# aask1357/hilcodec

Hardware: AMD Instinct MI355X
Metric: audio-seconds/sec (xRT) encode+RVQ+decode, 24 kHz batch=256 (higher is better)
Workload: dtype f32

## Files before the change

### hilcodec_amd/csrc/resblock_cfg.h

```cpp
#pragma once
#include <stdlib.h>

#include <atomic>
#include <type_traits>

#include "gemm_core.h"

using namespace hilc;

namespace {

constexpr int DWS = 12;

#ifndef HILC_RES_SHARE2_0
#define HILC_RES_SHARE2_0 0.61
#endif
#ifndef HILC_RES_SHARE3_0
#define HILC_RES_SHARE3_0 0.44
#define HILC_RES_SHARE3_1 0.31
#endif
template <int C, bool STREAM, bool SCARRY_ = false, int NB_ = 1, bool W8_ = false, int DR_ = 0, bool POST_ = false, bool SPEC0_ = false>
struct Cfg {
  static constexpr bool POST = POST_;
  static constexpr bool SPEC0 = SPEC0_;
  static_assert(!SPEC0_ || (C == 64 && (!STREAM || SCARRY_) && !W8_ && DR_ >= 0), "stage-0 input phase: the C = 64 encoder stage in the carry form (four waves, 128-column tiles)");
  static_assert(!POST_ || ((!STREAM || SCARRY_) && DR_ <= 0 && C <= 192 && !W8_), "closing conv: the carry form of a narrow stage (offline, or a hop's runs of whole streams)");
  static constexpr int NB = NB_;
  static constexpr int DR = DR_ > 0 ? DR_ : 0;
  static constexpr int UR = DR_ < 0 ? -DR_ : 0;
  static_assert(DR_ <= 0 || (((DR_ == 2 || DR_ == 4) && (!STREAM || SCARRY_) && C <= 192) || ((!STREAM || SCARRY_) && DR_ == 5 && C == 256) || (!SCARRY_ && DR_ == 8 && C == 512)),
                "down-sampling phase: carry form, r = 2 / 4 (C <= 192) or the wide encoder stages (C = 256: r = 5, offline and the hop's 32-column carry form; C = 512: r = 8, offline and a hop's whole-stream tiles)");
  static constexpr int DCAR = DR_ <= 0 ? 0 : (DR_ == 5 ? 12 : (DR_ == 8 ? 8 : 4));
  static_assert(DR_ >= 0 || ((DR_ == -8 && C >= 512) || (DR_ == -5 && C == 384) || ((DR_ == -4 || DR_ == -2) && C <= 192 && (!STREAM || SCARRY_))),
                "up-sampling phase: 32-column tiles (r = 8: whole streams, or the offline carry form), the C = 384 stage (r = 5) or the carry form (r = 4 / 2)");
  static constexpr int CH = C;
  static constexpr int CB = C / 32;
  static constexpr bool NARROW = C >= 256;
  static constexpr bool N32 = STREAM && SCARRY_ && NARROW;
  static_assert(!N32 || C == 256 || C == 384, "32-column carry form: the C = 256 / C = 384 stages of a hop");
  static constexpr int NCOL = NARROW ? ((C >= 512 || N32) ? 32 : 64) : 128;
  static constexpr int XS = NCOL + ((!STREAM || SCARRY_) ? 8 * NB_ + 2 * DCAR + (POST_ ? 4 : 0) : 0);
  static constexpr bool CARRYMODE = !STREAM || SCARRY_;
  static constexpr int HALO = CARRYMODE ? 0 : ((NARROW && C >= 512) ? 0 : 8);
  static constexpr int TO = NCOL - HALO;
  static constexpr int NW = (N32 && C == 384) ? 12 : ((C >= 192 || W8_) ? 8 : 4);
  static constexpr int NT = 64 * NW;
  static constexpr int RH = NW / (NCOL / 32);
  static constexpr int CBW = CB / RH;
  static constexpr int RPI = 256 / NCOL;
  static constexpr int RSTEP = RPI * NW;
  static constexpr int RW = C / RSTEP;
#ifndef HILC_RES_RB
#define HILC_RES_RB 4
#endif
  static constexpr int RB = HILC_RES_RB;
#ifdef HILC_RES_KP
  static constexpr int KP = HILC_RES_KP;
  static constexpr int DEPTH = HILC_RES_DEPTH;
#else
  static constexpr int KP = C >= 96 ? 4 : 8;
  static constexpr int DEPTH = C >= 256 ? 4 : (C == 128 ? (STREAM ? 2 : 3) : 2);
#endif
#ifndef HILC_RES_MINW
#define HILC_RES_MINW 2
#endif
  static constexpr int MINW = NW >= 8 ? NW / 4 : HILC_RES_MINW;
  static_assert(NW % (NCOL / 32) == 0 && CB % RH == 0 && RW % RB == 0 && C % RSTEP == 0, "tile split");
  static_assert(NB_ >= 1 && NB_ <= 3 && (NB_ == 1 || CARRYMODE || (NARROW && C >= 512)), "a chain needs carries or whole-stream tiles");
};

struct ResBlk {
  const float* w1t;
  const float* dw1_w;
  const float* dw1_b;
  const float* w2t;
  const float* dw2_w;
  const float* dw2_b;
  const float* hist1;
  const float* hist2;
  float* hist1_out;
  float* hist2_out;
  float pre_scale, out_scale;
};

struct ResUp {
  const float* xin;
  const float* tr_w;
  const float* w_lo;
  const float* w_hi;
  const float* bias;
  const float* hist;
  float* hist_out;
  float in_scale;
};

struct ResDown {
  const float* w_lo;
  const float* w_hi;
  const float* dw_w;
  const float* dw_b;
  const float* hist;
  float* hist_out;
  const float* res;
  float* y;
  float in_scale;
};

struct ResPost {
  const float* w;
  const float* bias;
  float* wav;
  const float* hist;
  float* hist_out;
  float in_scale, out_scale;
  int do_tanh;
};

struct ResSpec0 {
  const float* wav;
  const float* dft;
  const float* nyq;
  const float* pw;
  const float* bias;
  const float* pre_w;
  const float* pre_b;
  const float* hist;
  int hist_len;
  float pre_in_scale, mean, stdv, out_scale;
  int normalize;
};

constexpr int POST_CLASSES = 8;

constexpr int MAXBLK = 3;
constexpr int DDS = 12;

struct ResArgs {
  const float* x;
  ResBlk blk[MAXBLK];
  int nblk;
  ResDown dn;
  ResUp up;
  ResPost post;
  ResSpec0 spec;
  long run_tiles;
  float* y;
  int T, tiles;
  int classes;
  unsigned cum[5];
  long total_tiles;
  int B;
  unsigned div_magic, div_shift;
  int* sched;
  unsigned long long* dbg;
};

#ifdef HILC_DEBUG_STAMPS
unsigned long long* g_dbg = nullptr;
#endif

}
```

### hilcodec_amd/csrc/resblock_kernel.h

```cpp
#pragma once
#include "resblock_gemm.h"
#include "stream_gemm.h"

namespace {

struct Cols {
  long b;
  int t;
  int t_in;
  unsigned boff;
  unsigned hoff;
  int head, tail;
};
static_assert(sizeof(Cols) == 32, "no padding");

template <int C, bool STREAM, bool SCARRY = false, int NB = 1, bool W8 = false, int DRU = 0, bool POST = false, bool SPEC0 = false>
__global__ __launch_bounds__((Cfg<C, STREAM, SCARRY, NB, W8, DRU, POST, SPEC0>::NT), (Cfg<C, STREAM, SCARRY, NB, W8, DRU, POST, SPEC0>::MINW)) void resblock_kernel(ResArgs a) {
  using K = Cfg<C, STREAM, SCARRY, NB, W8, DRU, POST, SPEC0>;
  constexpr int DR = K::DR, UR = K::UR;
  using Pipe = WeightPipe<K>;
  constexpr int CBW = K::CBW, NW = K::NW, NT = K::NT, RW = K::RW, RB = K::RB, XS = K::XS, TO = K::TO, RSTEP = K::RSTEP;
  __shared__ __attribute__((aligned(16))) float Xbuf[4 + C * XS];
  constexpr bool DW_RELOAD = NB > 1 && K::NARROW && (4 + C * XS + NB * C * DWS) * 4 > 156 * 1024;
  __shared__ __attribute__((aligned(16))) float DW[(DW_RELOAD ? 1 : NB) * C * DWS];
  constexpr bool DWIDE = DR == 5 || DR == 8;
  __shared__ __attribute__((aligned(16))) float DWD[(DR > 0 && !DWIDE) ? 2 * C * DDS : 4];
  __shared__ __attribute__((aligned(16))) float HS[(STREAM && !K::NARROW) ? 2 * C * 4 : 4];
  __shared__ __attribute__((aligned(16))) float PR[POST ? POST_CLASSES * K::NCOL : 4];
  static_assert(!POST || (K::RPI * K::NW == POST_CLASSES), "a row class of the closing conv = the rows one half-wave walks");
  __shared__ __attribute__((aligned(16))) float SEG[SPEC0 ? (STREAM ? 256 : 192) : 4];
  __shared__ __attribute__((aligned(16))) float SEGS[SPEC0 ? (STREAM ? 256 : 192) : 4];
  float* const X = Xbuf + 4;
  const int tid = threadIdx.x, lane = tid & 63;
  const int wave = __builtin_amdgcn_readfirstlane(tid >> 6);
  constexpr int NCB = K::NCOL / 32;
  const int colblk = wave % NCB;
  const int wclass = wave / NCB;
  const int rowblk0 = wclass * CBW;
#if defined(HILC_DEBUG_WAVE_STAMPS)
  constexpr int WS_MAXB = 48;
  unsigned long long* ws_base = nullptr;
  int ws_k = 0;
#define STAMP(i) do { } while (0)
#define lds_barrier() do {                                                                                          \
    const unsigned long long t0_ = __builtin_amdgcn_s_memtime();                                                   \
    asm volatile("s_waitcnt lgkmcnt(0)" ::: "memory");                                                             \
    const unsigned long long t1_ = __builtin_amdgcn_s_memtime();                                                   \
    asm volatile("s_waitcnt lgkmcnt(0)\n\ts_barrier" ::: "memory");                                                 \
    const unsigned long long t2_ = __builtin_amdgcn_s_memtime();                                                   \
    if (ws_base != nullptr && lane == 0 && ws_k < WS_MAXB - 1) {                                                   \
      ws_base[ws_k * 3] = t0_; ws_base[ws_k * 3 + 1] = t1_; ws_base[ws_k * 3 + 2] = t2_;                           \
    }                                                                                                              \
    ++ws_k;                                                                                                        \
  } while (0)
#elif defined(HILC_DEBUG_STAMPS)
#define STAMP(i) do { if (a.dbg && tid == 0) a.dbg[stamp_tile * 8 + (i)] = __builtin_amdgcn_s_memtime(); } while (0)
  long stamp_tile = blockIdx.x;
#else
#define STAMP(i) do { } while (0)
#endif
  const int T = a.T;
  const int nblk = NB == 1 ? 1 : a.nblk;
  auto load_taps = [&](const ResBlk& bq, float* dst) {
    if constexpr (DW_RELOAD && !STREAM) {
      constexpr int NE = C * DWS;
      static_assert(NE % NT == 0, "whole rounds");
#pragma unroll
      for (int i = 0; i < NE / NT; ++i) {
        const int e = tid + i * NT;
        const int m = e / DWS, j = e - m * DWS;
        const float* src = j < 5 ? bq.dw1_w + (m * 5 + j) : (j == 5 ? bq.dw1_b + m : (j < 11 ? bq.dw2_w + (m * 5 + (j - 6)) : bq.dw2_b + m));
        dst[e] = *src;
      }
    } else if constexpr (DW_RELOAD) {
      constexpr int NE = C * DWS;
      static_assert(NE % NT == 0, "whole rounds");
#pragma unroll 3
      for (int i = 0; i < NE / NT; ++i) {
        const int e = tid + i * NT;
        const int m = e / DWS, j = e - m * DWS;
        const float* src = j < 5 ? bq.dw1_w + (m * 5 + j) : (j == 5 ? bq.dw1_b + m : (j < 11 ? bq.dw2_w + (m * 5 + (j - 6)) : bq.dw2_b + m));
        dst[e] = *src;
      }
    }
  };
  if constexpr (!DW_RELOAD) {
    constexpr int RND = (C + NT - 1) / NT;
    if constexpr (NB == 1 && STREAM) {
      const ResBlk& bq = a.blk[0];
#pragma unroll
      for (int it = 0; it < RND; ++it) {
        const int m = tid + it * NT;
        const int mc = (C % NT == 0 || m < C) ? m : C - 1;
#pragma unroll
        for (int w4 = 0; w4 < DWS / 4; ++w4) {
          float t4[4];
#pragma unroll
          for (int e = 0; e < 4; ++e) {
            const int j = 4 * w4 + e;
            t4[e] = j < 5 ? bq.dw1_w[mc * 5 + j] : (j == 5 ? bq.dw1_b[mc] : (j < 11 ? bq.dw2_w[mc * 5 + (j - 6)] : bq.dw2_b[mc]));
          }
          if (C % NT == 0 || m < C) *reinterpret_cast<f32x4*>(&DW[m * DWS + 4 * w4]) = f32x4{t4[0], t4[1], t4[2], t4[3]};
          __builtin_amdgcn_sched_barrier(0);
        }
      }
    } else {
    float tv[NB][RND][DWS];
#pragma unroll
    for (int q = 0; q < NB; ++q) {
      if (q < nblk) {
        const ResBlk& bq = a.blk[q];
#pragma unroll
        for (int it = 0; it < RND; ++it) {
          const int m = tid + it * NT;
          const int mc = (C % NT == 0 || m < C) ? m : C - 1;
#pragma unroll
          for (int j = 0; j < 5; ++j) tv[q][it][j] = bq.dw1_w[mc * 5 + j];
          tv[q][it][5] = bq.dw1_b[mc];
#pragma unroll
          for (int j = 0; j < 5; ++j) tv[q][it][6 + j] = bq.dw2_w[mc * 5 + j];
          tv[q][it][11] = bq.dw2_b[mc];
        }
      }
    }
#pragma unroll
    for (int q = 0; q < NB; ++q) {
      if (q < nblk) {
#pragma unroll
        for (int it = 0; it < RND; ++it) {
          const int m = tid + it * NT;
          if (C % NT == 0 || m < C) {
#pragma unroll
            for (int w4 = 0; w4 < DWS / 4; ++w4)
              *reinterpret_cast<f32x4*>(&DW[(q * C + m) * DWS + 4 * w4]) =
                  f32x4{tv[q][it][4 * w4], tv[q][it][4 * w4 + 1], tv[q][it][4 * w4 + 2], tv[q][it][4 * w4 + 3]};
          }
        }
      }
    }
    }
  }
  if constexpr (DR > 0 && !DWIDE) {
    constexpr int RND = (2 * C + NT - 1) / NT;
    float tw[RND][2 * DR + 1];
#pragma unroll
    for (int it = 0; it < RND; ++it) {
      const int m = tid + it * NT;
      const int mc = ((2 * C) % NT == 0 || m < 2 * C) ? m : 2 * C - 1;
#pragma unroll
      for (int j = 0; j < 2 * DR; ++j) tw[it][j] = a.dn.dw_w[mc * 2 * DR + j];
      tw[it][2 * DR] = a.dn.dw_b[mc];
    }
#pragma unroll
    for (int it = 0; it < RND; ++it) {
      const int m = tid + it * NT;
      if ((2 * C) % NT == 0 || m < 2 * C) {
#pragma unroll
        for (int j = 0; j < DDS; ++j) DWD[m * DDS + j] = j < 2 * DR ? tw[it][j] : (j == 8 ? tw[it][2 * DR] : 0.f);
      }
    }
  }
  if (tid < 4) Xbuf[tid] = 0.f;
  const int rsub = wave * K::RPI + (K::RPI > 1 ? lane / (K::NCOL / 4) : 0);
  const int c4 = (lane & (K::NCOL / 4 - 1)) * 4;
  [[maybe_unused]] const unsigned row_b = (unsigned)T * 4u;
  [[maybe_unused]] const bool one_head = STREAM && !K::NARROW && T >= K::NCOL;

  auto columns_of = [&](long tile) -> Cols {
    Cols s;
    s.boff = 0; s.hoff = 0; s.head = false; s.tail = false;
    if constexpr (STREAM) {
      const int flat = (int)tile * TO - K::HALO + c4;
      s.t_in = flat >= 0 && flat < a.B * T;
      const unsigned ub = s.t_in ? __umulhi((unsigned)flat, a.div_magic) >> a.div_shift : 0u;
      s.b = ub;
      s.t = s.t_in ? flat - (int)ub * T : 0;
      s.boff = (ub * (unsigned)(C * T) + (unsigned)s.t) * 4u;
      s.hoff = ub * (unsigned)(C * 4);
      s.head = s.t_in && s.t == 0;
      s.tail = s.t_in && c4 >= K::HALO && s.t == T - 4;
    } else {
      s.b = tile / a.tiles;
      s.t = (int)(tile - s.b * a.tiles) * TO + c4;
      s.t_in = s.t >= 0 && s.t < T;
    }
    return s;
  };
  auto xrow = [&](const Cols& s, int m) -> const f32x4* {
    if constexpr (STREAM)
      return reinterpret_cast<const f32x4*>(reinterpret_cast<const char*>(a.x) + (s.boff + (unsigned)m * row_b));
    else
      return reinterpret_cast<const f32x4*>(a.x + s.b * (long)C * T + (long)m * T + (s.t_in ? s.t : 0));
  };
  auto yrow = [&](const Cols& s, int m) -> f32x4* {
    if constexpr (STREAM)
      return reinterpret_cast<f32x4*>(reinterpret_cast<char*>(a.y) + (s.boff + (unsigned)m * row_b));
    else
      return reinterpret_cast<f32x4*>(a.y + s.b * (long)C * T + (long)m * T + s.t);
  };

  [[maybe_unused]] const float* hb0 = a.x;
  [[maybe_unused]] const float* hb1 = a.x;
  [[maybe_unused]] bool hv0 = false, hv1 = false;
  [[maybe_unused]] int blk_off = 0;
  Cols cs;
  const bool lane0 = c4 == 0, lane_last = c4 == K::NCOL - 4;
  auto prev_base = [&](int which) -> lptr_t {
    if constexpr (!K::CARRYMODE) return (lptr_t)(X + rsub * XS + c4 - 4);
    else return lane0 ? (lptr_t)(X + rsub * XS + K::NCOL + which * 4 + blk_off) : (lptr_t)(X + rsub * XS + c4 - 4);
  };
  auto prevs_of = [&](lptr_t pb, int m0, int which, f32x4 (&prev)[K::RB]) {
    if constexpr (!STREAM) {
// ... 505 lines not shown
      carry_out(xp6, 1, cur);
      if constexpr (STREAM) {
        if (cs.tail && !warm && bp.hist2_out != nullptr) {
#pragma unroll
          for (int i = 0; i < RB; ++i)
            *reinterpret_cast<f32x4*>(bp.hist2_out + cs.hoff + (rsub + RSTEP * (i0 + i)) * 4) = cur[i];
        }
      }
#pragma unroll
      for (int i = 0; i < RB; ++i) {
        const int m = rsub + RSTEP * (i0 + i);
        const float v[8] = {prev[i].x, prev[i].y, prev[i].z, prev[i].w, cur[i].x, cur[i].y, cur[i].z, cur[i].w};
        const float w[5] = {wb[i].x, wb[i].y, wc[i].x, wc[i].y, wc[i].z};
        f32x4 o;
#pragma unroll
        for (int e = 0; e < 4; ++e) {
          float s = 0.f;
#pragma unroll
          for (int j = 0; j < 5; ++j) s = fmaf(w[j], v[e + j], s);
          s = __fmul_rn(__fadd_rn(s, wc[i].w), bp.out_scale);
          o[e] = __fadd_rn(s, xr[i0 + i][e]);
        }
        if constexpr (NB == 1 && DR == 0 && !POST) {
          if (out_ok) *yrow(cs, m) = o;
        } else {
          if (last_blk) {
            if (out_ok) *yrow(cs, m) = o;
          } else if (post_blk) {
            *(lvec_t)(xp6 + i * RSTEP * XS) = prologue4v(o, a.post.in_scale, 1);
          } else {
            xr[i0 + i] = o;
          }
        }
      }
      if (UR == 0 && !SPEC0 && last_blk && have_next) {
#pragma unroll
        for (int i = 0; i < RB; ++i) xr[i0 + i] = *xrow(cn, rsub + RSTEP * (i0 + i));
      }
      xp6 += RB * RSTEP * XS;
      pb6 += RB * RSTEP * XS;
      asm volatile("" : "+v"(xp6), "+v"(pb6));
      __builtin_amdgcn_sched_barrier(0);
    }
    STAMP(7);
    lds_barrier();
    if (last_blk) cs = cn;
    }
    if constexpr (POST) {
      const bool have_next = next_tile < run1;
      const Cols cn = columns_of(have_next ? next_tile : tile);
      constexpr int PSLOT = K::NCOL + 8 * NB;
      float part[4] = {0.f, 0.f, 0.f, 0.f};
      lptr_t xq = (lptr_t)(X + rsub * XS + c4);
      lptr_t pq = lane0 ? (lptr_t)(X + rsub * XS + PSLOT) : (lptr_t)(X + rsub * XS + c4 - 4);
      const float* wq = a.post.w + rsub * 5;
      [[maybe_unused]] bool any_head = false;
      [[maybe_unused]] const float* hq = a.post.w;
      [[maybe_unused]] float* hqo = nullptr;
      [[maybe_unused]] bool qtail = false;
      if constexpr (STREAM) {
        const int first = (int)tile * TO, last = first + K::NCOL - 1;
        const unsigned bl = __umulhi((unsigned)last, a.div_magic) >> a.div_shift;
        any_head = (int)bl * T >= first || first % T == 0;
        if (a.post.hist != nullptr) hq = a.post.hist + cs.hoff + rsub * 4;
        qtail = cs.tail && !warm && a.post.hist_out != nullptr;
        if (a.post.hist_out != nullptr) hqo = a.post.hist_out + cs.hoff + rsub * 4;
      }
#pragma nounroll
      for (int i0 = 0; i0 < RW; i0 += RB) {
        f32x4 cur[RB], prev[RB];
        float w[RB][5];
#pragma unroll
        for (int i = 0; i < RB; ++i) {
          cur[i] = *(lvec_t)(xq + i * RSTEP * XS);
          prev[i] = *(lvec_t)(pq + i * RSTEP * XS);
#pragma unroll
          for (int j = 0; j < 5; ++j) w[i][j] = wq[i * RSTEP * 5 + j];
        }
        wq += RB * RSTEP * 5;
        if constexpr (STREAM) {
          if (any_head) {
            f32x4 hv[RB];
#pragma unroll
            for (int i = 0; i < RB; ++i)
              hv[i] = a.post.hist != nullptr ? *reinterpret_cast<const f32x4*>(hq + i * RSTEP * 4) : f32x4{0.f, 0.f, 0.f, 0.f};
#pragma unroll
            for (int i = 0; i < RB; ++i)
#pragma unroll
              for (int e = 0; e < 4; ++e) prev[i][e] = cs.head ? hv[i][e] : prev[i][e];
          }
          if (qtail) {
#pragma unroll
            for (int i = 0; i < RB; ++i) *reinterpret_cast<f32x4*>(hqo + i * RSTEP * 4) = cur[i];
          }
          hq += a.post.hist != nullptr ? RB * RSTEP * 4 : 0;
          hqo += RB * RSTEP * 4;
        }
        if (lane_last) {
#pragma unroll
          for (int i = 0; i < RB; ++i) *(lvec_t)(xq + i * RSTEP * XS + 4 + 8 * NB) = cur[i];
        }
#pragma unroll
        for (int i = 0; i < RB; ++i) {
          const float v[8] = {prev[i].x, prev[i].y, prev[i].z, prev[i].w, cur[i].x, cur[i].y, cur[i].z, cur[i].w};
#pragma unroll
          for (int e = 0; e < 4; ++e)
#pragma unroll
            for (int j = 0; j < 5; ++j) part[e] = fmaf(w[i][j], v[e + j], part[e]);
        }
        xq += RB * RSTEP * XS;
        pq += RB * RSTEP * XS;
        asm volatile("" : "+v"(xq), "+v"(pq));
        __builtin_amdgcn_sched_barrier(0);
      }
      *reinterpret_cast<f32x4*>(&PR[rsub * K::NCOL + c4]) = f32x4{part[0], part[1], part[2], part[3]};
      lds_barrier();
      if (tid < K::NCOL) {
        float sacc = PR[tid];
#pragma unroll
        for (int q = 1; q < POST_CLASSES; ++q) sacc = __fadd_rn(sacc, PR[q * K::NCOL + tid]);
        if (a.post.bias != nullptr) sacc = __fadd_rn(sacc, a.post.bias[0]);
        sacc = __fmul_rn(sacc, a.post.out_scale);
        if (a.post.do_tanh) sacc = tanhf(sacc);
        if constexpr (STREAM) {
          const long flat = (long)tile * TO + tid;
          if (!warm && flat < (long)a.B * T) a.post.wav[flat] = sacc;
        } else {
          const int t = cs.t - c4 + tid;
          if (!warm && t < T) a.post.wav[cs.b * (long)T + t] = sacc;
        }
      }
      cs = cn;
    }
    if constexpr (DR > 0) {
      const ResDown& dn = a.dn;
      const bool have_next = next_tile < run1;
      const Cols cn = columns_of(have_next ? next_tile : tile);
      const float* wd0 = dn.w_lo + (long)wclass * (C * C / K::RH);
      const float* wd1 = dn.w_hi + (long)wclass * (C * C / K::RH);
      asm volatile("" : "+s"(wd0), "+s"(wd1));
      Pipe wp;
      wp.prefetch(wd0, lane);
      auto d0 = [&]() {
        lptr_t xp = (lptr_t)(X + rsub * XS + c4);
#pragma unroll
        for (int i0 = 0; i0 < RW; i0 += RB) {
#pragma unroll
          for (int i = 0; i < RB; ++i)
            *(lvec_t)(xp + i * RSTEP * XS) = prologue4v(zero_unless(cs.t_in, xr[i0 + i]), dn.in_scale, 1);
          xp += RB * RSTEP * XS;
          asm volatile("" : "+v"(xp));
        }
      };
      d0();
      if (!DWIDE && !SPEC0 && have_next) {
#pragma unroll
        for (int i = 0; i < RW; ++i) xr[i] = *xrow(cn, rsub + RSTEP * i);
      }
      lds_barrier();
      f32x16 acc0[CBW];
      [[maybe_unused]] f32x16 acc1[DWIDE ? 1 : CBW];
      if constexpr (K::NARROW) gemm_phase_rolled<K>(wd0, X, acc0, wp, colblk, lane);
      else gemm_phase<K>(wd0, X, acc0, wp, colblk, lane);
      if constexpr (!DWIDE) {
        wp.prefetch(wd1, lane);
        if constexpr (K::NARROW) gemm_phase_rolled<K>(wd1, X, acc1, wp, colblk, lane);
        else gemm_phase<K>(wd1, X, acc1, wp, colblk, lane);
      }
      const bool out_ok = !warm && (STREAM ? cs.t_in : cs.t < T);
      [[maybe_unused]] const bool out_ok_tile = !warm;
      const int To = T / DR;
#pragma unroll
      for (int h = 0; h < 2; ++h) {
        if constexpr (DWIDE) {
          if (h == 1) {
            lds_barrier();
            wp.prefetch(wd1, lane);
            d0();
            if (have_next) {
#pragma unroll
              for (int i = 0; i < RW; ++i) xr[i] = *xrow(cn, rsub + RSTEP * i);
            }
            lds_barrier();
            gemm_phase_rolled<K>(wd1, X, acc0, wp, colblk, lane);
          }
        }
        lds_barrier();
        if constexpr (DWIDE) acc_to_x<K>(acc0, X, rowblk0, colblk, lane);
        else acc_to_x<K>(h ? acc1 : acc0, X, rowblk0, colblk, lane);
        lds_barrier();
        if constexpr (DWIDE) {
          constexpr int DC = K::DCAR;
          constexpr int DOFF = K::NCOL + 8 * NB;
          constexpr bool SLOTS = K::CARRYMODE;
          const int jl = c4 >> 2;
          const int t0 = STREAM ? (int)tile * TO : cs.t - c4;
          const int o = t0 / DR + jl;
          const int base = o * DR - DR - t0;
          [[maybe_unused]] unsigned sb = 0;
          int os = o;
          if constexpr (STREAM) {
            const bool in = o < a.B * To;
            sb = in ? __umulhi((unsigned)(o * DR), a.div_magic) >> a.div_shift : 0u;
            os = in ? o - (int)sb * To : 1;
          }
          [[maybe_unused]] const bool dhead = STREAM && os == 0;
          const bool act = out_ok_tile && (STREAM ? o < a.B * To : o < To) && o * DR + DR - 1 < t0 + K::NCOL;
          [[maybe_unused]] const int slot = DOFF + DC * h + DC;
          lptr_t rowp = (lptr_t)(X + rsub * XS);
          const float* wrow = dn.dw_w + (long)(h * C + rsub) * (2 * DR);
          const float* brow = dn.dw_b + (h * C + rsub);
          float wn[2 * DR], bn;
          [[maybe_unused]] float hn[STREAM ? DR : 1];
          [[maybe_unused]] const float* hrow = dn.dw_w;
          [[maybe_unused]] float* horow = nullptr;
          [[maybe_unused]] const bool use_hist = STREAM && dn.hist != nullptr;
          if constexpr (STREAM) {
            if (use_hist) hrow = dn.hist + ((long)sb * (2 * C) + h * C + rsub) * DR;
            if (dn.hist_out != nullptr) horow = dn.hist_out + ((long)cs.b * (2 * C) + h * C + rsub) * DR;
          }
          [[maybe_unused]] const bool dtail = STREAM && cs.tail && !warm && dn.hist_out != nullptr;
          auto taps_of = [&](const float* wr, const float* br) {
            if constexpr (DR == 8) {
#pragma unroll
              for (int q = 0; q < 4; ++q) {
                const f32x4 w4 = *reinterpret_cast<const f32x4*>(wr + 4 * q);
#pragma unroll
                for (int e = 0; e < 4; ++e) wn[4 * q + e] = w4[e];
              }
            } else {
#pragma unroll
              for (int q = 0; q < DR; ++q) {
                const f32x2 w2 = *reinterpret_cast<const f32x2*>(wr + 2 * q);
                wn[2 * q] = w2.x; wn[2 * q + 1] = w2.y;
              }
            }
            bn = br[0];
            if constexpr (STREAM) {
              if (use_hist) {
                if constexpr (DR == 8) {
#pragma unroll
                  for (int q = 0; q < 2; ++q) {
                    const f32x4 h4 = *reinterpret_cast<const f32x4*>(hrow + 4 * q);
#pragma unroll
                    for (int e = 0; e < 4; ++e) hn[4 * q + e] = h4[e];
                  }
                } else {
#pragma unroll
                  for (int j = 0; j < DR; ++j) hn[j] = hrow[j];
                }
              } else {
#pragma unroll
                for (int j = 0; j < DR; ++j) hn[j] = 0.f;
              }
            }
          };
          taps_of(wrow, brow);
          long yo = STREAM ? ((long)sb * (2 * C) + h * C + rsub) * (long)To + os : ((long)cs.b * (2 * C) + h * C + rsub) * (long)To + o;
#pragma nounroll
          for (int i0 = 0; i0 < RW; ++i0) {
            float v[2 * DR], w[2 * DR];
#pragma unroll
            for (int j = 0; j < 2 * DR; ++j) w[j] = wn[j];
            const float bb = bn;
            [[maybe_unused]] float hc[STREAM ? DR : 1];
            if constexpr (STREAM) {
#pragma unroll
              for (int j = 0; j < DR; ++j) hc[j] = hn[j];
            }
            wrow += RSTEP * (2 * DR);
            brow += RSTEP;
            if constexpr (STREAM) hrow += use_hist ? RSTEP * DR : 0;
            if (i0 + 1 < RW) taps_of(wrow, brow);
            if constexpr (DR == 8) {
#pragma unroll
              for (int q = 0; q < 4; ++q) {
                const int col = base + 4 * q;
                const f32x4 x4 = *(lvec_t)(rowp + (col >= 0 ? col : (SLOTS ? slot + col : 0)));
#pragma unroll
                for (int e = 0; e < 4; ++e) v[4 * q + e] = x4[e];
              }
            } else {
#pragma unroll
              for (int j = 0; j < 2 * DR; ++j) {
                const int col = base + j;
                v[j] = *(rowp + (col >= 0 ? col : (SLOTS ? slot + col : 0)));
              }
            }
            if constexpr (STREAM) {
#pragma unroll
              for (int j = 0; j < DR; ++j) v[j] = dhead ? hc[j] : v[j];
            }
            const f32x4 keep = *(lvec_t)(rowp + c4);
            if constexpr (STREAM) {
              const f32x4 before = *(lvec_t)(rowp + (c4 >= 4 ? c4 - 4 : 0));
              if (dtail) {
                if constexpr (DR == 8) {
                  *reinterpret_cast<f32x4*>(horow) = before;
                  *reinterpret_cast<f32x4*>(horow + 4) = keep;
                } else {
                  horow[0] = before.w; horow[1] = keep.x; horow[2] = keep.y; horow[3] = keep.z; horow[4] = keep.w;
                }
              }
              horow += RSTEP * DR;
            }
            if constexpr (SLOTS) {
              if (c4 >= K::NCOL - DC)
                *(lvec_t)(rowp + DOFF + DC * h + (c4 - (K::NCOL - DC))) = keep;
            }
            float s0 = 0.f;
#pragma unroll
            for (int j = 0; j < 2 * DR; ++j) s0 = fmaf(w[j], v[j], s0);
            s0 = __fadd_rn(s0, bb);
            if (act) dn.y[yo] = dn.res != nullptr ? __fadd_rn(s0, dn.res[yo]) : s0;
            yo += (long)RSTEP * To;
            rowp += RSTEP * XS;
          }
        } else {
        lptr_t xpd = (lptr_t)(X + rsub * XS + c4);
        lptr_t pbd = lane0 ? (lptr_t)(X + rsub * XS + K::NCOL + 8 * NB + 4 * h) : (lptr_t)(X + rsub * XS + c4 - 4);
#pragma unroll
        for (int i0 = 0; i0 < RW; i0 += RB) {
          f32x4 cur[RB], prev[RB], wa[RB], wb[RB];
          float bb[RB];
#pragma unroll
          for (int i = 0; i < RB; ++i) {
            const int m = h * C + rsub + RSTEP * (i0 + i);
            cur[i] = *(lvec_t)(xpd + i * RSTEP * XS);
            prev[i] = *(lvec_t)(pbd + i * RSTEP * XS);
            wa[i] = *reinterpret_cast<const f32x4*>(&DWD[m * DDS]);
            if constexpr (DR == 4) wb[i] = *reinterpret_cast<const f32x4*>(&DWD[m * DDS + 4]);
            bb[i] = DWD[m * DDS + 8];
          }
          if constexpr (STREAM) {
            const unsigned hro = (unsigned)cs.b * (unsigned)(2 * C * DR) + (unsigned)(h * C + rsub + RSTEP * i0) * DR;
#pragma unroll
            for (int i = 0; i < RB; ++i) {
              f32x4 hv = {0.f, 0.f, 0.f, 0.f};
              if (dn.hist != nullptr) {
                const float* hp = dn.hist + (cs.t_in ? hro + (unsigned)(RSTEP * i * DR) : 0u);
                if constexpr (DR == 4) hv = *reinterpret_cast<const f32x4*>(hp);
                else { const f32x2 h2 = *reinterpret_cast<const f32x2*>(hp); hv = f32x4{0.f, 0.f, h2.x, h2.y}; }
              }
#pragma unroll
              for (int e = 0; e < 4; ++e) prev[i][e] = cs.head ? hv[e] : prev[i][e];
            }
          }
          if (lane_last) {
#pragma unroll
            for (int i = 0; i < RB; ++i) *(lvec_t)(xpd + i * RSTEP * XS + 4 + 8 * NB + 4 * h) = cur[i];
          }
          if constexpr (STREAM) {
            if (cs.tail && !warm && dn.hist_out != nullptr) {
              const unsigned hro = (unsigned)cs.b * (unsigned)(2 * C * DR) + (unsigned)(h * C + rsub + RSTEP * i0) * DR;
#pragma unroll
              for (int i = 0; i < RB; ++i) {
                float* hp = dn.hist_out + hro + (unsigned)(RSTEP * i * DR);
                if constexpr (DR == 4) *reinterpret_cast<f32x4*>(hp) = cur[i];
                else *reinterpret_cast<f32x2*>(hp) = f32x2{cur[i].z, cur[i].w};
              }
            }
          }
#pragma unroll
          for (int i = 0; i < RB; ++i) {
            const int m = h * C + rsub + RSTEP * (i0 + i);
            const long yo = ((long)cs.b * (2 * C) + m) * (long)To + (cs.t_in ? cs.t / DR : 0);
            if constexpr (DR == 4) {
              const float v[8] = {prev[i].x, prev[i].y, prev[i].z, prev[i].w, cur[i].x, cur[i].y, cur[i].z, cur[i].w};
              const float w[8] = {wa[i].x, wa[i].y, wa[i].z, wa[i].w, wb[i].x, wb[i].y, wb[i].z, wb[i].w};
              float s0 = 0.f;
#pragma unroll
              for (int j = 0; j < 8; ++j) s0 = fmaf(w[j], v[j], s0);
              s0 = __fadd_rn(s0, bb[i]);
              if (out_ok) dn.y[yo] = dn.res != nullptr ? __fadd_rn(s0, dn.res[yo]) : s0;
            } else {
              const float v[6] = {prev[i].z, prev[i].w, cur[i].x, cur[i].y, cur[i].z, cur[i].w};
              const float w[4] = {wa[i].x, wa[i].y, wa[i].z, wa[i].w};
              f32x2 o2;
#pragma unroll
              for (int e = 0; e < 2; ++e) {
                float s0 = 0.f;
#pragma unroll
                for (int j = 0; j < 4; ++j) s0 = fmaf(w[j], v[2 * e + j], s0);
                o2[e] = __fadd_rn(s0, bb[i]);
              }
              if (out_ok) {
                if (dn.res != nullptr) {
                  const f32x2 r2 = *reinterpret_cast<const f32x2*>(dn.res + yo);
                  o2[0] = __fadd_rn(o2[0], r2.x);
                  o2[1] = __fadd_rn(o2[1], r2.y);
                }
                *reinterpret_cast<f32x2*>(dn.y + yo) = o2;
              }
            }
          }
          xpd += RB * RSTEP * XS;
          pbd += RB * RSTEP * XS;
          asm volatile("" : "+v"(xpd), "+v"(pbd));
          __builtin_amdgcn_sched_barrier(0);
        }
        }
      }
      lds_barrier();
      cs = cn;
    }
    tile = next_tile;
  }
  if (!K::CARRYMODE && K::NW == 4 && a.sched != nullptr && tid == 0) {
    if (atomicAdd(a.sched + 1, 1) == (int)gridDim.x - 1) {
      a.sched[0] = 0;
      a.sched[1] = 0;
    }
  }
  if (touch == 1.2345678e-30f) a.y[0] = touch;
#if defined(HILC_DEBUG_WAVE_STAMPS)
  if (ws_base != nullptr && lane == 0) ws_base[(WS_MAXB - 1) * 3 + 1] = (unsigned long long)ws_k;
#undef lds_barrier
#endif
#undef STAMP
}

}
```

Measured before the change: 3510.

## Prefetch downsample residual early and batch wide depthwise taps in offline path

```diff
diff --git a/hilcodec_amd/csrc/resblock_cfg.h b/hilcodec_amd/csrc/resblock_cfg.h
--- a/hilcodec_amd/csrc/resblock_cfg.h
+++ b/hilcodec_amd/csrc/resblock_cfg.h
@@ -33,6 +33,12 @@
   static constexpr int DCAR = DR_ <= 0 ? 0 : (DR_ == 5 ? 12 : (DR_ == 8 ? 8 : 4));
   static_assert(DR_ >= 0 || ((DR_ == -8 && C >= 512) || (DR_ == -5 && C == 384) || ((DR_ == -4 || DR_ == -2) && C <= 192 && (!STREAM || SCARRY_))),
                 "up-sampling phase: 32-column tiles (r = 8: whole streams, or the offline carry form), the C = 384 stage (r = 5) or the carry form (r = 4 / 2)");
+  static constexpr int DWB = DR_ == 8 ? 1 : 2;
+  static constexpr int DPF = 1;
+#ifndef HILC_RES_DRES_EARLY
+#define HILC_RES_DRES_EARLY 1
+#endif
+  static constexpr bool DRES_EARLY = DR_ > 0 && HILC_RES_DRES_EARLY;
   static constexpr int CH = C;
   static constexpr int CB = C / 32;
   static constexpr bool NARROW = C >= 256;
diff --git a/hilcodec_amd/csrc/resblock_down_index.h b/hilcodec_amd/csrc/resblock_down_index.h
--- /dev/null
+++ b/hilcodec_amd/csrc/resblock_down_index.h
@@ -0,0 +1,24 @@
+#pragma once
+#if defined(__HIPCC__) || defined(__CUDACC__)
+#define HILC_DN_HD __host__ __device__ inline
+#else
+#define HILC_DN_HD inline
+#endif
+
+namespace hilc_down {
+
+HILC_DN_HD long out_index(long b, int C, int m, int To, int col) { return (b * (2 * C) + m) * (long)To + col; }
+
+struct WideLane {
+  int o, base, act;
+};
+HILC_DN_HD WideLane wide_lane(int t0, int jl, int r, int ncol, int To, bool warm) {
+  WideLane w;
+  w.o = t0 / r + jl;
+  w.base = w.o * r - r - t0;
+  w.act = !warm && w.o < To && w.o * r + r - 1 < t0 + ncol;
+  return w;
+}
+HILC_DN_HD int wide_col(const WideLane& w) { return w.act ? w.o : 0; }
+
+}
diff --git a/hilcodec_amd/csrc/resblock_kernel.h b/hilcodec_amd/csrc/resblock_kernel.h
--- a/hilcodec_amd/csrc/resblock_kernel.h
+++ b/hilcodec_amd/csrc/resblock_kernel.h
@@ -1,4 +1,5 @@
 #pragma once
+#include "resblock_down_index.h"
 #include "resblock_gemm.h"
 #include "stream_gemm.h"
 
@@ -54,10 +55,18 @@
     ++ws_k;                                                                                                        \
   } while (0)
 #elif defined(HILC_DEBUG_STAMPS)
-#define STAMP(i) do { if (a.dbg && tid == 0) a.dbg[stamp_tile * 8 + (i)] = __builtin_amdgcn_s_memtime(); } while (0)
+#ifndef HILC_STAMP_SLOTS
+#define HILC_STAMP_SLOTS 8
+#endif
+#define STAMP(i) do { if (a.dbg && tid == 0) a.dbg[stamp_tile * HILC_STAMP_SLOTS + (i)] = __builtin_amdgcn_s_memtime(); } while (0)
   long stamp_tile = blockIdx.x;
 #else
 #define STAMP(i) do { } while (0)
+#endif
+#if defined(HILC_DEBUG_STAMPS) && !defined(HILC_DEBUG_WAVE_STAMPS) && HILC_STAMP_SLOTS >= 24
+#define DSTAMP(i) STAMP(8 + (i))
+#else
+#define DSTAMP(i) do { } while (0)
 #endif
   const int T = a.T;
   const int nblk = NB == 1 ? 1 : a.nblk;
@@ -869,23 +878,50 @@
           asm volatile("" : "+v"(xp));
         }
       };
+      [[maybe_unused]] const int Tow = T / DR;
+      [[maybe_unused]] const bool have_res = dn.res != nullptr && !warm;
+      constexpr bool DPRE = DWIDE && !STREAM;
+      [[maybe_unused]] float rr[DPRE ? RW : 1] = {};
+      [[maybe_unused]] hilc_down::WideLane wl = {0, 0, 0};
+      [[maybe_unused]] long yo0 = 0;
+      if constexpr (DPRE) {
+        const int t0 = cs.t - c4;
+        wl = hilc_down::wide_lane(t0, c4 >> 2, DR, K::NCOL, Tow, warm);
+        yo0 = hilc_down::out_index(cs.b, C, rsub, Tow, hilc_down::wide_col(wl));
+      }
+      auto res_fetch = [&](int h) {
+        if constexpr (DPRE) {
+          if (have_res) {
+            const float* rp = dn.res + (yo0 + (long)h * C * Tow);
+#pragma unroll
+            for (int i = 0; i < RW; ++i) {
+              rr[i] = rp[0];
+              rp += (long)RSTEP * Tow;
+            }
+          }
+        }
+      };
       d0();
       if (!DWIDE && !SPEC0 && have_next) {
 #pragma unroll
         for (int i = 0; i < RW; ++i) xr[i] = *xrow(cn, rsub + RSTEP * i);
       }
+      if constexpr (K::DRES_EARLY) res_fetch(0);
       lds_barrier();
+      DSTAMP(0);
       f32x16 acc0[CBW];
       [[maybe_unused]] f32x16 acc1[DWIDE ? 1 : CBW];
       if constexpr (K::NARROW) gemm_phase_rolled<K>(wd0, X, acc0, wp, colblk, lane);
       else gemm_phase<K>(wd0, X, acc0, wp, colblk, lane);
+      DSTAMP(1);
       if constexpr (!DWIDE) {
         wp.prefetch(wd1, lane);
         if constexpr (K::NARROW) gemm_phase_rolled<K>(wd1, X, acc1, wp, colblk, lane);
         else gemm_phase<K>(wd1, X, acc1, wp, colblk, lane);
-      }
-      const bool out_ok = !warm && (STREAM ? cs.t_in : cs.t < T);
-      [[maybe_unused]] const bool out_ok_tile = !warm;
+        DSTAMP(2);
+      }
+      if constexpr (!K::DRES_EARLY) res_fetch(0);
+      [[maybe_unused]] const bool out_ok = !warm && (STREAM ? cs.t_in : cs.t < T);
       const int To = T / DR;
 #pragma unroll
       for (int h = 0; h < 2; ++h) {
@@ -898,140 +934,234 @@
 #pragma unroll
               for (int i = 0; i < RW; ++i) xr[i] = *xrow(cn, rsub + RSTEP * i);
             }
+            if constexpr (K::DRES_EARLY) res_fetch(1);
             lds_barrier();
+            DSTAMP(9);
             gemm_phase_rolled<K>(wd1, X, acc0, wp, colblk, lane);
+            DSTAMP(2);
+            if constexpr (!K::DRES_EARLY) res_fetch(1);
           }
         }
         lds_barrier();
+        DSTAMP(3 + 3 * h);
         if constexpr (DWIDE) acc_to_x<K>(acc0, X, rowblk0, colblk, lane);
         else acc_to_x<K>(h ? acc1 : acc0, X, rowblk0, colblk, lane);
         lds_barrier();
+        DSTAMP(4 + 3 * h);
         if constexpr (DWIDE) {
           constexpr int DC = K::DCAR;
           constexpr int DOFF = K::NCOL + 8 * NB;
           constexpr bool SLOTS = K::CARRYMODE;
-          const int jl = c4 >> 2;
-          const int t0 = STREAM ? (int)tile * TO : cs.t - c4;
-          const int o = t0 / DR + jl;
-          const int base = o * DR - DR - t0;
-          [[maybe_unused]] unsigned sb = 0;
-          int os = o;
           if constexpr (STREAM) {
-            const bool in = o < a.B * To;
-            sb = in ? __umulhi((unsigned)(o * DR), a.div_magic) >> a.div_shift : 0u;
-            os = in ? o - (int)sb * To : 1;
-          }
-          [[maybe_unused]] const bool dhead = STREAM && os == 0;
-          const bool act = out_ok_tile && (STREAM ? o < a.B * To : o < To) && o * DR + DR - 1 < t0 + K::NCOL;
-          [[maybe_unused]] const int slot = DOFF + DC * h + DC;
-          lptr_t rowp = (lptr_t)(X + rsub * XS);
-          const float* wrow = dn.dw_w + (long)(h * C + rsub) * (2 * DR);
-          const float* brow = dn.dw_b + (h * C + rsub);
-          float wn[2 * DR], bn;
-          [[maybe_unused]] float hn[STREAM ? DR : 1];
-          [[maybe_unused]] const float* hrow = dn.dw_w;
-          [[maybe_unused]] float* horow = nullptr;
-          [[maybe_unused]] const bool use_hist = STREAM && dn.hist != nullptr;
-          if constexpr (STREAM) {
-            if (use_hist) hrow = dn.hist + ((long)sb * (2 * C) + h * C + rsub) * DR;
-            if (dn.hist_out != nullptr) horow = dn.hist_out + ((long)cs.b * (2 * C) + h * C + rsub) * DR;
-          }
-          [[maybe_unused]] const bool dtail = STREAM && cs.tail && !warm && dn.hist_out != nullptr;
-          auto taps_of = [&](const float* wr, const float* br) {
-            if constexpr (DR == 8) {
-#pragma unroll
-              for (int q = 0; q < 4; ++q) {
-                const f32x4 w4 = *reinterpret_cast<const f32x4*>(wr + 4 * q);
-#pragma unroll
-                for (int e = 0; e < 4; ++e) wn[4 * q + e] = w4[e];
-              }
-            } else {
-#pragma unroll
-              for (int q = 0; q < DR; ++q) {
-                const f32x2 w2 = *reinterpret_cast<const f32x2*>(wr + 2 * q);
-                wn[2 * q] = w2.x; wn[2 * q + 1] = w2.y;
-              }
+            const int jl = c4 >> 2;
+            const int t0 = STREAM ? (int)tile * TO : cs.t - c4;
+            const int o = t0 / DR + jl;
+            const int base = o * DR - DR - t0;
+            [[maybe_unused]] unsigned sb = 0;
+            int os = o;
+            if constexpr (STREAM) {
+              const bool in = o < a.B * To;
+              sb = in ? __umulhi((unsigned)(o * DR), a.div_magic) >> a.div_shift : 0u;
+              os = in ? o - (int)sb * To : 1;
             }
-            bn = br[0];
+            [[maybe_unused]] const bool dhead = STREAM && os == 0;
+            const bool act = !warm && (STREAM ? o < a.B * To : o < To) && o * DR + DR - 1 < t0 + K::NCOL;
+            [[maybe_unused]] const int slot = DOFF + DC * h + DC;
+            lptr_t rowp = (lptr_t)(X + rsub * XS);
+            const float* wrow = dn.dw_w + (long)(h * C + rsub) * (2 * DR);
+            const float* brow = dn.dw_b + (h * C + rsub);
+            float wn[2 * DR], bn;
+            [[maybe_unused]] float hn[STREAM ? DR : 1];
+            [[maybe_unused]] const float* hrow = dn.dw_w;
+            [[maybe_unused]] float* horow = nullptr;
+            [[maybe_unused]] const bool use_hist = STREAM && dn.hist != nullptr;
             if constexpr (STREAM) {
-              if (use_hist) {
-                if constexpr (DR == 8) {
-#pragma unroll
-                  for (int q = 0; q < 2; ++q) {
-                    const f32x4 h4 = *reinterpret_cast<const f32x4*>(hrow + 4 * q);
-#pragma unroll
-                    for (int e = 0; e < 4; ++e) hn[4 * q + e] = h4[e];
+              if (use_hist) hrow = dn.hist + ((long)sb * (2 * C) + h * C + rsub) * DR;
+              if (dn.hist_out != nullptr) horow = dn.hist_out + ((long)cs.b * (2 * C) + h * C + rsub) * DR;
+            }
+            [[maybe_unused]] const bool dtail = STREAM && cs.tail && !warm && dn.hist_out != nullptr;
+            auto taps_of = [&](const float* wr, const float* br) {
+              if constexpr (DR == 8) {
+#pragma unroll
+                for (int q = 0; q < 4; ++q) {
+                  const f32x4 w4 = *reinterpret_cast<const f32x4*>(wr + 4 * q);
+#pragma unroll
+                  for (int e = 0; e < 4; ++e) wn[4 * q + e] = w4[e];
+                }
+              } else {
+#pragma unroll
+                for (int q = 0; q < DR; ++q) {
+                  const f32x2 w2 = *reinterpret_cast<const f32x2*>(wr + 2 * q);
+                  wn[2 * q] = w2.x; wn[2 * q + 1] = w2.y;
+                }
+              }
+              bn = br[0];
+              if constexpr (STREAM) {
+                if (use_hist) {
+                  if constexpr (DR == 8) {
+#pragma unroll
+                    for (int q = 0; q < 2; ++q) {
+                      const f32x4 h4 = *reinterpret_cast<const f32x4*>(hrow + 4 * q);
+#pragma unroll
+                      for (int e = 0; e < 4; ++e) hn[4 * q + e] = h4[e];
+                    }
+                  } else {
+#pragma unroll
+                    for (int j = 0; j < DR; ++j) hn[j] = hrow[j];
                   }
                 } else {
 #pragma unroll
-                  for (int j = 0; j < DR; ++j) hn[j] = hrow[j];
+                  for (int j = 0; j < DR; ++j) hn[j] = 0.f;
+                }
+              }
+            };
+            taps_of(wrow, brow);
+            long yo = STREAM ? ((long)sb * (2 * C) + h * C + rsub) * (long)To + os : ((long)cs.b * (2 * C) + h * C + rsub) * (long)To + o;
+#pragma nounroll
+            for (int i0 = 0; i0 < RW; ++i0) {
+              float v[2 * DR], w[2 * DR];
+#pragma unroll
+              for (int j = 0; j < 2 * DR; ++j) w[j] = wn[j];
+              const float bb = bn;
+              [[maybe_unused]] float hc[STREAM ? DR : 1];
+              if constexpr (STREAM) {
+#pragma unroll
+                for (int j = 0; j < DR; ++j) hc[j] = hn[j];
+              }
+              wrow += RSTEP * (2 * DR);
+              brow += RSTEP;
+              if constexpr (STREAM) hrow += use_hist ? RSTEP * DR : 0;
+              if (i0 + 1 < RW) taps_of(wrow, brow);
+              if constexpr (DR == 8) {
+#pragma unroll
+                for (int q = 0; q < 4; ++q) {
+                  const int col = base + 4 * q;
+                  const f32x4 x4 = *(lvec_t)(rowp + (col >= 0 ? col : (SLOTS ? slot + col : 0)));
+#pragma unroll
+                  for (int e = 0; e < 4; ++e) v[4 * q + e] = x4[e];
                 }
               } else {
 #pragma unroll
-                for (int j = 0; j < DR; ++j) hn[j] = 0.f;
-              }
+                for (int j = 0; j < 2 * DR; ++j) {
+                  const int col = base + j;
+                  v[j] = *(rowp + (col >= 0 ? col : (SLOTS ? slot + col : 0)));
+                }
+              }
+              if constexpr (STREAM) {
+#pragma unroll
+                for (int j = 0; j < DR; ++j) v[j] = dhead ? hc[j] : v[j];
+              }
+              const f32x4 keep = *(lvec_t)(rowp + c4);
+              if constexpr (STREAM) {
+                const f32x4 before = *(lvec_t)(rowp + (c4 >= 4 ? c4 - 4 : 0));
+                if (dtail) {
+                  if constexpr (DR == 8) {
+                    *reinterpret_cast<f32x4*>(horow) = before;
+                    *reinterpret_cast<f32x4*>(horow + 4) = keep;
+                  } else {
+                    horow[0] = before.w; horow[1] = keep.x; horow[2] = keep.y; horow[3] = keep.z; horow[4] = keep.w;
+                  }
+                }
+                horow += RSTEP * DR;
+              }
+              if constexpr (SLOTS) {
+                if (c4 >= K::NCOL - DC)
+                  *(lvec_t)(rowp + DOFF + DC * h + (c4 - (K::NCOL - DC))) = keep;
+              }
+              float s0 = 0.f;
+#pragma unroll
+              for (int j = 0; j < 2 * DR; ++j) s0 = fmaf(w[j], v[j], s0);
+              s0 = __fadd_rn(s0, bb);
+              if (act) dn.y[yo] = dn.res != nullptr ? __fadd_rn(s0, dn.res[yo]) : s0;
+              yo += (long)RSTEP * To;
+              rowp += RSTEP * XS;
             }
-          };
-          taps_of(wrow, brow);
-          long yo = STREAM ? ((long)sb * (2 * C) + h * C + rsub) * (long)To + os : ((long)cs.b * (2 * C) + h * C + rsub) * (long)To + o;
-#pragma nounroll
-          for (int i0 = 0; i0 < RW; ++i0) {
-            float v[2 * DR], w[2 * DR];
-#pragma unroll
-            for (int j = 0; j < 2 * DR; ++j) w[j] = wn[j];
-            const float bb = bn;
-            [[maybe_unused]] float hc[STREAM ? DR : 1];
-            if constexpr (STREAM) {
-#pragma unroll
-              for (int j = 0; j < DR; ++j) hc[j] = hn[j];
+          } else {
+            const int base = wl.base;
+            const bool act = wl.act != 0;
+            [[maybe_unused]] const int slot = DOFF + DC * h + DC;
+            constexpr int WB = K::DWB, PF = K::DPF, NS = PF + 1;
+            static_assert(RW % WB == 0 && PF * WB < RW, "whole batches");
+            lptr_t rowp = (lptr_t)(X + rsub * XS);
+            const float* wrow = dn.dw_w + (long)(h * C + rsub) * (2 * DR);
+            const float* brow = dn.dw_b + (h * C + rsub);
+            float wn[NS][WB][2 * DR], bn[NS][WB];
+            auto taps_of = [&](int ns, int rn) {
+              const float* wr = wrow + rn * (2 * DR);
+              const float* br = brow + rn;
+#pragma unroll
+              for (int b = 0; b < WB; ++b) {
+                if constexpr (DR == 8) {
+#pragma unroll
+                  for (int q = 0; q < 4; ++q) {
+                    const f32x4 w4 = *reinterpret_cast<const f32x4*>(wr + b * RSTEP * (2 * DR) + 4 * q);
+#pragma unroll
+                    for (int e = 0; e < 4; ++e) wn[ns][b][4 * q + e] = w4[e];
+                  }
+                } else {
+#pragma unroll
+                  for (int q = 0; q < DR; ++q) {
+                    const f32x2 w2 = *reinterpret_cast<const f32x2*>(wr + b * RSTEP * (2 * DR) + 2 * q);
+                    wn[ns][b][2 * q] = w2.x; wn[ns][b][2 * q + 1] = w2.y;
+                  }
+                }
+                bn[ns][b] = br[b * RSTEP];
+              }
+            };
+#pragma unroll
+            for (int k = 0; k < PF; ++k) taps_of(k, k * WB * RSTEP);
+            float* const yp = dn.y + (yo0 + (long)h * C * To);
+            int ro = 0;
+#pragma unroll
+            for (int i0 = 0; i0 < RW; i0 += WB) {
+              const int kb = i0 / WB, cur = kb % NS;
+              float v[WB][2 * DR], w[WB][2 * DR], bb[WB];
+              if (i0 + PF * WB < RW) taps_of((kb + PF) % NS, ro + PF * WB * RSTEP);
+              f32x4 keep[WB];
+#pragma unroll
+              for (int b = 0; b < WB; ++b) {
+                const lptr_t rq = rowp + b * RSTEP * XS;
+                if constexpr (DR == 8) {
+#pragma unroll
+                  for (int q = 0; q < 4; ++q) {
+                    const int col = base + 4 * q;
+                    const f32x4 x4 = *(lvec_t)(rq + (col >= 0 ? col : (SLOTS ? slot + col : 0)));
+#pragma unroll
+                    for (int e = 0; e < 4; ++e) v[b][4 * q + e] = x4[e];
+                  }
+                } else {
+#pragma unroll
+                  for (int j = 0; j < 2 * DR; ++j) {
+                    const int col = base + j;
+                    v[b][j] = *(rq + (col >= 0 ? col : (SLOTS ? slot + col : 0)));
+                  }
+                }
+#pragma unroll
+                for (int j = 0; j < 2 * DR; ++j) w[b][j] = wn[cur][b][j];
+                bb[b] = bn[cur][b];
+                keep[b] = *(lvec_t)(rq + c4);
+              }
+              if constexpr (SLOTS) {
+                if (c4 >= K::NCOL - DC) {
+#pragma unroll
+                  for (int b = 0; b < WB; ++b)
+                    *(lvec_t)(rowp + b * RSTEP * XS + DOFF + DC * h + (c4 - (K::NCOL - DC))) = keep[b];
+                }
+              }
+#pragma unroll
+              for (int b = 0; b < WB; ++b) {
+                float s0 = 0.f;
+#pragma unroll
+                for (int j = 0; j < 2 * DR; ++j) s0 = fmaf(w[b][j], v[b][j], s0);
+                s0 = __fadd_rn(s0, bb[b]);
+                if (act) yp[(long)(ro + b * RSTEP) * To] = have_res ? __fadd_rn(s0, rr[i0 + b]) : s0;
+              }
+              rowp += WB * RSTEP * XS;
+              ro += WB * RSTEP;
+              asm volatile("" : "+v"(rowp));
+              asm volatile("" : "+s"(ro));
+              __builtin_amdgcn_sched_barrier(0);
             }
-            wrow += RSTEP * (2 * DR);
-            brow += RSTEP;
-            if constexpr (STREAM) hrow += use_hist ? RSTEP * DR : 0;
-            if (i0 + 1 < RW) taps_of(wrow, brow);
-            if constexpr (DR == 8) {
-#pragma unroll
-              for (int q = 0; q < 4; ++q) {
-                const int col = base + 4 * q;
-                const f32x4 x4 = *(lvec_t)(rowp + (col >= 0 ? col : (SLOTS ? slot + col : 0)));
-#pragma unroll
-                for (int e = 0; e < 4; ++e) v[4 * q + e] = x4[e];
-              }
-            } else {
-#pragma unroll
-              for (int j = 0; j < 2 * DR; ++j) {
-                const int col = base + j;
-                v[j] = *(rowp + (col >= 0 ? col : (SLOTS ? slot + col : 0)));
-              }
-            }
-            if constexpr (STREAM) {
-#pragma unroll
-              for (int j = 0; j < DR; ++j) v[j] = dhead ? hc[j] : v[j];
-            }
-            const f32x4 keep = *(lvec_t)(rowp + c4);
-            if constexpr (STREAM) {
-              const f32x4 before = *(lvec_t)(rowp + (c4 >= 4 ? c4 - 4 : 0));
-              if (dtail) {
-                if constexpr (DR == 8) {
-                  *reinterpret_cast<f32x4*>(horow) = before;
-                  *reinterpret_cast<f32x4*>(horow + 4) = keep;
-                } else {
-                  horow[0] = before.w; horow[1] = keep.x; horow[2] = keep.y; horow[3] = keep.z; horow[4] = keep.w;
-                }
-              }
-              horow += RSTEP * DR;
-            }
-            if constexpr (SLOTS) {
-              if (c4 >= K::NCOL - DC)
-                *(lvec_t)(rowp + DOFF + DC * h + (c4 - (K::NCOL - DC))) = keep;
-            }
-            float s0 = 0.f;
-#pragma unroll
-            for (int j = 0; j < 2 * DR; ++j) s0 = fmaf(w[j], v[j], s0);
-            s0 = __fadd_rn(s0, bb);
-            if (act) dn.y[yo] = dn.res != nullptr ? __fadd_rn(s0, dn.res[yo]) : s0;
-            yo += (long)RSTEP * To;
-            rowp += RSTEP * XS;
           }
         } else {
         lptr_t xpd = (lptr_t)(X + rsub * XS + c4);
@@ -1117,8 +1247,10 @@
           __builtin_amdgcn_sched_barrier(0);
         }
         }
+        DSTAMP(5 + 3 * h);
       }
       lds_barrier();
+      DSTAMP(10);
       cs = cn;
     }
     tile = next_tile;
@@ -1135,6 +1267,7 @@
 #undef lds_barrier
 #endif
 #undef STAMP
+#undef DSTAMP
 }
 
 }
```

After: 3521, median of 6. About the same (+0.3%).
